# cuteboyqq/DPVO

Hardware: AMD Instinct MI355X
Metric: update-iterations/sec (altcorr+fastba) on 96-patch/2048-edge graph, 1→8 GPU (higher is better)
Workload: dtype f32; 1 GPU; cfg2: 96 patches/frame x 2048 edges, p=3, 4-level pyramid [1, 2, 4, 8], fp32 features, BA 2 iters; patches_per_frame=96, edges=2048, frames=12, radius=3, channels=128, feature_ring=36, parallelism=replicas x1

## Files before the change

dpvo_amd/csrc/ba_window.hip:

```cpp
#include <unistd.h>

#include <algorithm>
#include <chrono>
#include <cstdio>
#include <random>
#include <cstdlib>
#include <map>
#include <mutex>

#include "ba_paths.hpp"
#include "ba_solve.hpp"
#include "pyr_insert.hpp"

namespace dpvo {
namespace {
using namespace bad;

constexpr int kWT = 256;
constexpr int kPT = 512;
constexpr int kWMaxN = 16;
constexpr int kWMaxE = 10240;
constexpr int kWMaxG = 256;
constexpr int kWLds = 160 * 1024;
constexpr int kHistMax = 12288;
constexpr int kWSlots = 64;
constexpr unsigned kFix = 0xFF;
constexpr unsigned kHbm = 0xFE;
constexpr int kChunk = 256;
constexpr int kPart = 42;
constexpr int kPartPad = 48;
constexpr int kGranPad = 48;
constexpr long long kSpin = 2000000;
constexpr int kEpochWord = kWMaxG;
constexpr int kFlagWords = kWMaxG + 8;
constexpr int kRefine = 1;
constexpr int kBufDword3 = 0x00020000;
constexpr int kSc1 = 16;

constexpr int kStChol = 1, kStClamp = 2, kStTimeout = 16, kStCap = 32;

typedef unsigned v4u __attribute__((ext_vector_type(4)));

constexpr int kWMaxNB = kWMaxN * (kWMaxN + 1) / 2;
constexpr int kPlanShardMax = 16;
constexpr int kMetaWork = 64;
constexpr size_t kMetaBytes = sizeof(int) * (kMetaWork + (size_t)kPlanShardMax * kWMaxNB);

struct Plan {
  int* epos;
  int* poff;
  unsigned* pmask;
  int* pkk;
  int* meta;
  int* status;
  int* sink;
  const int* t0d;
};

struct WArgs {
  float* poses;
  float* patches;
  const float* intrinsics;
  const float* target;
  const float* weight;
  const float* lmbda;
  const int64_t* ii;
  const int64_t* jj;
  const int64_t* kk;
  int E, P, num_poses, num_patches, t0, N, iters, NB, Sd, So, G;
  Plan plan;
  double* part;
  v4u* gran;
  long long* flags;
  float* ejg;
  int* status;
  int* sink;
  int64_t* marks;
  double* dxo;
  const int* t0d;
  unsigned long long salt;
};

__device__ __forceinline__ size_t al16(size_t v) { return (v + 15) & ~(size_t)15; }
typedef double f64x2 __attribute__((ext_vector_type(2)));

__device__ __forceinline__ int opaque_tid() {
  int t = threadIdx.x;
  asm volatile("" : "+v"(t));
  return t;
}

__device__ __forceinline__ void mark(const WArgs& A, int slot) {
  if (A.marks && blockIdx.x == 0 && threadIdx.x == 0) A.marks[slot] = (int64_t)wall_clock64();
}


__host__ __device__ constexpr int plan_cap(int E) { return (E + 15) & ~15; }
__host__ __device__ constexpr size_t plan_u_bytes(int cap) {
  size_t p2 = 1;
  while (p2 < (size_t)cap) p2 <<= 1;
  const size_t keys = p2 <= 8192 ? 8 * p2 : 4 * p2;
  return keys > 8 * (size_t)cap ? keys : 8 * (size_t)cap;
}
__host__ __device__ constexpr size_t plan_lds_bytes(int cap) {
  return 256 + 6 * (size_t)cap + (((size_t)cap + 15) & ~(size_t)15) + plan_u_bytes(cap);
}
static_assert(plan_lds_bytes(kWMaxE) <= (size_t)kWLds, "plan LDS");

__device__ __forceinline__ int bucket_rank(const unsigned short* s, int a, int b, int e) {
  int rank = 0;
  for (int t = a; t < b; t += 8) {
    int v[8];
#pragma unroll
    for (int k = 0; k < 8; k++) v[k] = s[min(t + k, b - 1)];
#pragma unroll
    for (int k = 0; k < 8; k++) rank += (t + k < b && v[k] < e) ? 1 : 0;
  }
  return rank;
}

constexpr int kPlanPer = kWMaxE / kPT;
template <int kPer = kPlanPer>
__device__ __forceinline__ void plan_edges_pass(const int64_t* __restrict__ ii,
                                                const int64_t* __restrict__ jj,
                                                const int64_t* __restrict__ kk, int E,
                                                int num_patches, int num_poses, int t0, int N,
                                                int* ctl, unsigned short* code, int (&kv)[kPer]) {
  const int tid = threadIdx.x, lane = tid & 63, T = kPT;
  const int kmaxc = num_patches - 1;
  if (tid == 0) {
    ctl[0] = 0x7fffffff;
    ctl[1] = -1;
    ctl[2] = 0x7fffffff;
    ctl[3] = 0;
  }
  __syncthreads();
  constexpr int kPlanRound = kPer % 5 == 0 ? 5 : kPer;
  static_assert(kPer % kPlanRound == 0, "load rounds");
  int kmin = 0x7fffffff, kmax = -1, fmin = 0x7fffffff, bad = 0;
#pragma unroll
  for (int r = 0; r < kPer; r++) kv[r] = 0;
  if (E > 0) {
#pragma unroll
    for (int r0 = 0; r0 < kPer; r0 += kPlanRound) {
      if (r0 * T >= E) break;
      int64_t vk[kPlanRound], vi[kPlanRound], vj[kPlanRound];
#pragma unroll
      for (int r = 0; r < kPlanRound; r++) {
// ... 53 lines not shown
__device__ __forceinline__ void plan_store_work(const Plan& plan, const int* wl, int s, int N) {
  const int nb = N * (N + 1) / 2;
  for (int t = threadIdx.x; t < nb; t += blockDim.x)
    plan.meta[kMetaWork + t * kPlanShardMax + s] = wl[t];
}

__device__ __forceinline__ void plan_block(const int64_t* __restrict__ ii,
                                           const int64_t* __restrict__ jj,
                                           const int64_t* __restrict__ kk, int E, int num_patches,
                                           int num_poses, int t0, int N, const Plan& plan,
                                           char* lds, int cap = kWMaxE) {
  if (plan.t0d) t0 = *plan.t0d;
  const int tid = threadIdx.x, T = kPT;
  const int kmaxc = num_patches - 1;
  int* ctl = (int*)lds;
  int* scr = ctl + 16;
  unsigned short* code = (unsigned short*)(lds + 256);
  unsigned short* key = code + cap;
  unsigned short* spos = key + cap;
  unsigned char* head = (unsigned char*)(spos + cap);
  char* U = (char*)head + al16(cap);
  int kv[kPlanPer];
  plan_edges_pass(ii, jj, kk, E, num_patches, num_poses, t0, N, ctl, code, kv);
  int kmin = ctl[0];
  const int R = ctl[1] - kmin + 1;
  if (R <= kHistMax && (size_t)(R + E) * 4 <= plan_u_bytes(cap) && E < (1 << 14)) {
    int* hist = (int*)U;
    unsigned* pm = reinterpret_cast<unsigned*>(hist + R);
    for (int v = tid; v < R; v += T) hist[v] = 0;
    for (int u = tid; u < E; u += T) pm[u] = 0u;
    __syncthreads();
#pragma unroll
    for (int r = 0; r < kPlanPer; r++) {
      const int e = tid + r * T;
      if (e < E) atomicAdd(&hist[kv[r] - kmin], 1);
    }
    __syncthreads();
    const int nuniq = fscan(hist, R, scr, 14) & 0x3fff;
#pragma unroll
    for (int r = 0; r < kPlanPer; r++) {
      const int e = tid + r * T;
      if (e >= E) continue;
      const int old = atomicAdd(&hist[kv[r] - kmin], 1 << 14);
      spos[old >> 14] = (unsigned short)e;
      const unsigned c = code[e], ci = c & 0xff, cj = c >> 8;
      const unsigned m = (ci != kFix ? 1u << ci : 0u) | (cj != kFix ? 1u << cj : 0u);
      if (m) atomicOr(&pm[old & 0x3fff], m);
    }
    __syncthreads();
#pragma unroll
    for (int r = 0; r < kPlanPer; r++) {
      const int e = tid + r * T;
      if (e >= E) continue;
      const int v = kv[r] - kmin, hv = hist[v];
      const int b = hv >> 14, a = (v == 0) ? 0 : (hist[v - 1] >> 14);
      const int rank = bucket_rank(spos, a, b, e);
      plan.epos[a + rank] = e;
      if (rank == 0) {
        const int u = hv & 0x3fff;
        plan.poff[u] = a;
        plan.pkk[u] = kv[r];
        plan.pmask[u] = pm[u];
      }
    }
    if (tid == 0) {
      plan.poff[nuniq] = E;
      plan.meta[0] = nuniq;
      plan.meta[1] = ctl[2];
      plan.meta[2] = ctl[3];
      plan.meta[3] = 0;
      if (ctl[3] && plan.sink) atomicOr(plan.sink, ctl[3]);
      *plan.status = 0;
    }
    return;
  }
  unsigned short* pos_edge = spos;
  if (R <= kHistMax && (size_t)R * 4 <= plan_u_bytes(cap)) {
    int* hist = (int*)U;
    for (int v = tid; v < R; v += T) hist[v] = 0;
    for (int p = tid; p < E; p += T) head[p] = 0;
    __syncthreads();
#pragma unroll
    for (int r = 0; r < kPlanPer; r++) {
      const int e = tid + r * T;
      if (e < E) atomicAdd(&hist[kv[r] - kmin], 1);
    }
    __syncthreads();
    fscan(hist, R, scr);
    for (int v = tid; v < R; v += T) {
      const int a = hist[v], b = (v + 1 < R) ? hist[v + 1] : E;
      if (b > a) head[a] = 1;
    }
    __syncthreads();
#pragma unroll
    for (int r = 0; r < kPlanPer; r++) {
      const int e = tid + r * T;
      if (e < E) spos[atomicAdd(&hist[kv[r] - kmin], 1)] = (unsigned short)e;
    }
    __syncthreads();
    int dst[kPlanPer];
#pragma unroll
    for (int r = 0; r < kPlanPer; r++) {
      const int e = tid + r * T;
      dst[r] = -1;
      if (e >= E) continue;
      const int v = kv[r] - kmin;
      const int b = hist[v], a = (v == 0) ? 0 : hist[v - 1];
      dst[r] = a + bucket_rank(spos, a, b, e);
    }
    __syncthreads();
// ... 20 lines not shown
          k32[e] = ((unsigned)min(kv[r] - kmin, (1 << 18) - 1) << 14) | (unsigned)e;
      }
    }
    for (int i = E + tid; i < P2; i += T) {
      if (wide)
        k64[i] = ~0ull;
      else
        k32[i] = ~0u;
    }
    __syncthreads();
    for (int size = 2; size <= P2; size <<= 1)
      for (int stride = size >> 1; stride > 0; stride >>= 1) {
        for (int i = tid; i < P2 / 2; i += T) {
          const int lo = 2 * i - (i & (stride - 1));
          const int hi = lo + stride;
          const bool up = ((lo & size) == 0);
          if (wide) {
            const unsigned long long a = k64[lo], b = k64[hi];
            if ((a > b) == up) {
              k64[lo] = b;
              k64[hi] = a;
            }
          } else {
            const unsigned a = k32[lo], b = k32[hi];
            if ((a > b) == up) {
              k32[lo] = b;
              k32[hi] = a;
            }
          }
        }
        __syncthreads();
      }
    for (int p = tid; p < E; p += T) {
      if (wide) {
        spos[p] = (unsigned short)(k64[p] & 0xffffffffull);
        head[p] = (p == 0 || (k64[p] >> 32) != (k64[p - 1] >> 32)) ? 1 : 0;
      } else {
        spos[p] = (unsigned short)(k32[p] & 0x3fffu);
        head[p] = (p == 0 || (k32[p] >> 14) != (k32[p - 1] >> 14)) ? 1 : 0;
      }
    }
  }
  __syncthreads();
  int* hd = (int*)U;
  for (int p = tid; p < E; p += T) hd[p] = head[p];
  __syncthreads();
  const int nuniq = fscan(hd, E, scr);
  for (int p = tid; p < E; p += T) {
    const int u1 = (p + 1 < E) ? hd[p + 1] : nuniq;
    const bool is_head = u1 != hd[p];
    const int u = u1 - 1;
    const int e = pos_edge[p];
    plan.epos[p] = e;
    if (is_head) {
      plan.poff[u] = p;
      plan.pkk[u] = (int)min(max(kk[e], (int64_t)0), (int64_t)kmaxc);
    }
  }
  if (tid == 0) plan.poff[nuniq] = E;
  unsigned* mask = (unsigned*)(U + sizeof(int) * cap);
  for (int u = tid; u < nuniq; u += T) mask[u] = 0u;
  __syncthreads();
  for (int p = tid; p < E; p += T) {
    const int u = ((p + 1 < E) ? hd[p + 1] : nuniq) - 1;
    const unsigned c = code[pos_edge[p]];
    const unsigned ci = c & 0xff, cj = c >> 8;
    const unsigned m = (ci != kFix ? 1u << ci : 0u) | (cj != kFix ? 1u << cj : 0u);
    if (m) atomicOr(&mask[u], m);
  }
  __syncthreads();
  for (int u = tid; u < nuniq; u += T) plan.pmask[u] = mask[u];
  if (tid == 0) {
    plan.meta[0] = nuniq;
    plan.meta[1] = ctl[2];
    plan.meta[2] = ctl[3];
    plan.meta[3] = 0;
    if (ctl[3] && plan.sink) atomicOr(plan.sink, ctl[3]);
    *plan.status = 0;
  }
}

__host__ __device__ constexpr int plan_shards(int E) {
  return E <= 512 ? 1 : ((E + 511) / 512 < kPlanShardMax ? (E + 511) / 512 : kPlanShardMax);
}
template <int kPer>
__device__ __forceinline__ void plan_sharded_k(const int64_t* __restrict__ ii,
                                             const int64_t* __restrict__ jj,
                                               const int64_t* __restrict__ kk, int E, int num_patches,
                                               int num_poses, int t0, int N, const Plan& plan,
                                               char* lds, int cap, size_t lds_bytes, int s, int S) {
  if (S <= 1) {
    if (s == 0) plan_block(ii, jj, kk, E, num_patches, num_poses, t0, N, plan, lds, cap);
    return;
  }
  if (plan.t0d) t0 = *plan.t0d;
  auto stamp = [&](int q) {
    if (s == 0 && threadIdx.x == 0) {
      reinterpret_cast<int64_t*>(plan.meta + 16)[q] = (int64_t)wall_clock64();
      if (q == 0 || q == 6) reinterpret_cast<int64_t*>(plan.meta + 16)[7 + (q == 6)] = (int64_t)clock64();
    }
  };
  stamp(0);
  const int tid = threadIdx.x, lane = tid & 63, wid = tid >> 6, T = kPT;
  int* ctl = (int*)lds;
  int* scr = ctl + 16;
  unsigned short* spos = (unsigned short*)(lds + 256);
// ... 80 lines not shown
    }
    return;
  }
  const int lo = (int)((long long)R * s / S), hi = (int)((long long)R * (s + 1) / S), nl = hi - lo;
  const int per = (R + T - 1) / T, v0 = tid * per, v1 = min(v0 + per, R);
  int sum = 0;
  for (int k0 = v0; k0 < v1; k0 += 4) {
    int c[4];
#pragma unroll
    for (int j = 0; j < 4; j++) c[j] = hf[(kmin + min(k0 + j, v1 - 1)) & zm];
#pragma unroll
    for (int j = 0; j < 4; j++) sum += k0 + j < v1 ? (c[j] << 14) | (c[j] > 0 ? 1 : 0) : 0;
  }
  const int incl = wave_incl_sum(sum);
  if (lane == 63) scr[wid] = incl;
  lds_barrier();
  int total = 0, run = incl - sum;
#pragma unroll
  for (int w = 0; w < kPT / 64; w++) {
    const int x = scr[w];
    total += x;
    run += w < wid ? x : 0;
  }
  for (int k0 = v0; k0 < v1; k0 += 4) {
    int c[4];
#pragma unroll
    for (int j = 0; j < 4; j++) c[j] = hf[(kmin + min(k0 + j, v1 - 1)) & zm];
#pragma unroll
    for (int j = 0; j < 4; j++) {
      const int v = k0 + j;
      if (v >= v1) continue;
      if (v >= lo && v < hi) hf[(kmin + v) & zm] = run;
      if (v == lo) ctl[4] = run >> 14;
      if (v == hi) ctl[5] = run >> 14;
      run += (c[j] << 14) | (c[j] > 0 ? 1 : 0);
    }
  }
  lds_barrier();
  stamp(3);
  const int nuniq = total & 0x3fff;
  const int below = ctl[4], top = hi < R ? ctl[5] : total >> 14;
#pragma unroll
  for (int r = 0; r < kPer; r++) {
    const int e = tid + r * T;
    const int v = kv[r] - kmin - lo;
    if (e >= E || v < 0 || v >= nl) continue;
    const int p = atomicAdd(&hf[kv[r] & zm], 1 << 14) >> 14;
    spos[p] = (unsigned short)e;
    sv[p] = (unsigned short)v;
    if (mk[r]) atomicOr(&pm[v], mk[r]);
  }
  lds_barrier();
  stamp(4);
  plan_block_work(nl, [&](int v, int& c, unsigned& m) {
    c = (hf[(kmin + lo + v) & zm] >> 14) - (v == 0 ? below : (hf[(kmin + lo + v - 1) & zm] >> 14));
    m = pm[v];
  }, wl);
  stamp(5);
  for (int p = below + tid; p < top; p += T) {
    const int e = spos[p], v = sv[p];
    const int hv = hf[(kmin + lo + v) & zm];
    const int b = hv >> 14, a = v == 0 ? below : (hf[(kmin + lo + v - 1) & zm] >> 14);
    const int rank = bucket_rank(spos, a, b, e);
    plan.epos[a + rank] = e;
    if (rank == 0) {
      const int u = hv & 0x3fff;
      plan.poff[u] = a;
      plan.pkk[u] = kmin + lo + v;
      plan.pmask[u] = pm[v];
    }
  }
  lds_barrier();
  plan_store_work(plan, wl, s, N);
  if (tid == 0 && s == S - 1) plan.poff[nuniq] = E;
  if (tid == 0 && s == 0) {
    plan.meta[0] = nuniq;
    plan.meta[1] = ctl[2];
    plan.meta[2] = ctl[3];
    plan.meta[3] = S;
    if (ctl[3] && plan.sink) atomicOr(plan.sink, ctl[3]);
    *plan.status = 0;
  }
  stamp(6);
}

__device__ __forceinline__ void plan_sharded_long(const int64_t* __restrict__ ii,
                                               const int64_t* __restrict__ jj,
                                               const int64_t* __restrict__ kk, int E, int num_patches,
                                               int num_poses, int t0, int N, const Plan& plan,
                                               char* lds, int cap, size_t lds_bytes, int s, int S) {
  plan_sharded_k<kPlanPer>(ii, jj, kk, E, num_patches, num_poses, t0, N, plan, lds, cap, lds_bytes,
                           s, S);
}
__device__ __forceinline__ void plan_sharded(const int64_t* __restrict__ ii,
                                             const int64_t* __restrict__ jj,
                                             const int64_t* __restrict__ kk, int E, int num_patches,
                                             int num_poses, int t0, int N, const Plan& plan,
                                             char* lds, int cap, size_t lds_bytes, int s, int S) {
  if (__builtin_expect(E <= 4 * kPT, 1))
    plan_sharded_k<4>(ii, jj, kk, E, num_patches, num_poses, t0, N, plan, lds, cap, lds_bytes, s, S);
  else
    plan_sharded_long(ii, jj, kk, E, num_patches, num_poses, t0, N, plan, lds, cap, lds_bytes, s, S);
}

__global__ void __launch_bounds__(kPT) ba_plan_kernel(const int64_t* __restrict__ ii,
                                                      const int64_t* __restrict__ jj,
                                                      const int64_t* __restrict__ kk, int E,
                                                      int num_patches, int num_poses, int t0, int N,
                                                      Plan plan) {
  extern __shared__ __attribute__((aligned(16))) char lds[];
  plan_sharded(ii, jj, kk, E, num_patches, num_poses, t0, N, plan, lds, kWMaxE, kWLds, blockIdx.x,
               gridDim.x);
}

struct RArgs {
  const float* poses;
  const float* patches;
// ... 115 lines not shown
      const float4* e4 = reinterpret_cast<const float4*>(ej + 12 * (size_t)q);
      e0 = e4[0];
      e1 = e4[1];
      e2 = e4[2];
    } else {
      const __amdgpu_buffer_rsrc_t rs = __builtin_amdgcn_make_buffer_rsrc(
          const_cast<float*>(ejg), 0, (int)(sizeof(float) * 24 * (size_t)E), kBufDword3);
      const int o = (int)(sizeof(float) * 12 * ((size_t)par * E + eid[q]));
      e0 = __builtin_bit_cast(float4, __builtin_amdgcn_raw_buffer_load_b128(rs, o, 0, kSc1));
      e1 = __builtin_bit_cast(float4, __builtin_amdgcn_raw_buffer_load_b128(rs, o + 16, 0, kSc1));
      e2 = __builtin_bit_cast(float4, __builtin_amdgcn_raw_buffer_load_b128(rs, o + 32, 0, kSc1));
    }
  }
};

enum { cNrel = 0, cNrp = 1, cFmin = 2, cFail = 3, cTimeout = 4, cCap = 5, cFailAny = 6, cLMulti = 7,
       cScan = 16 };

__device__ __forceinline__ double edges_etdx(const WL& L, const WArgs& A, int q0, int q1, int par,
                                             int N) {
  constexpr int kEb = 4;
  double ex = 0.0;
  for (int qb = q0; qb < q1; qb += kEb) {
    float4 e[kEb][3];
    unsigned cc[kEb];
#pragma unroll
    for (int u = 0; u < kEb; u++) {
      const int q = min(qb + u, q1 - 1);
      cc[u] = L.ec[q];
      L.ld_ej(A.ejg, A.E, q, par, e[u][0], e[u][1], e[u][2]);
    }
#pragma unroll
    for (int u = 0; u < kEb; u++) {
      const bool live = qb + u < q1;
      const unsigned si = cc[u] & 0xff, sj = cc[u] >> 8;
      const unsigned nm = (unsigned)max(N - 1, 0);
      const double* dj = L.dX + 6 * min(sj, nm);
      const double* di = L.dX + 6 * min(si, nm);
      const float4 e0 = e[u][0], e1 = e[u][1], e2 = e[u][2];
      const double tj = (double)e0.x * dj[0] + (double)e0.y * dj[1] + (double)e0.z * dj[2] +
                        (double)e0.w * dj[3] + (double)e1.x * dj[4] + (double)e1.y * dj[5];
      const double ti = (double)e1.z * di[0] + (double)e1.w * di[1] + (double)e2.x * di[2] +
                        (double)e2.y * di[3] + (double)e2.z * di[4] + (double)e2.w * di[5];
      ex += (live && sj < (unsigned)N) ? tj : 0.0;
      ex += (live && si < (unsigned)N) ? ti : 0.0;
    }
  }
  return ex;
}
__device__ __forceinline__ double patch_etdx(const WL& L, const WArgs& A, int ri, int par, int N) {
  return edges_etdx(L, A, L.roff[ri], L.roff[ri + 1], par, N);
}

__device__ __forceinline__ unsigned wslot(int gp, int t0, int N, int fmin) {
  if (gp >= t0 && gp < t0 + N) return (unsigned)(gp - t0);
  const int k = gp - fmin;
  return (k >= 0 && k < kWSlots - N) ? (unsigned)(N + k) : kHbm;
}

__device__ __forceinline__ void pose_of(const WArgs& A, const WL& L, unsigned slot, int gp,
                                        float* P) {
  if (slot != kHbm) {
    const float4 a0 = *reinterpret_cast<const float4*>(L.pose + 8 * slot);
    const float4 a1 = *reinterpret_cast<const float4*>(L.pose + 8 * slot + 4);
    P[0] = a0.x; P[1] = a0.y; P[2] = a0.z; P[3] = a0.w; P[4] = a1.x; P[5] = a1.y; P[6] = a1.z;
  } else {
    const float* g = A.poses + 7 * (size_t)gp;
#pragma unroll
    for (int k = 0; k < 7; k++) P[k] = g[k];
  }
}

template <int MODE>
__device__ void assemble(const WArgs& A, const WL& L, int nrel, int a, int b, double lam,
                         float fx, float fy, float cx, float cy, int par, double* acc,
                         int& nact) {
  nact = 0;
  constexpr int NA = (MODE == 1) ? 27 : (MODE == 2 ? 36 : 1);
  const int tid = opaque_tid(), N = A.N;
  const unsigned ua = (unsigned)a, ub = (unsigned)b;
  double* pe = reinterpret_cast<double*>(L.region);
#pragma unroll
  for (int k = 0; k < NA; k++) acc[k] = 0.0;
  for (int pa = 0; pa < nrel;) {
    int pb = pa + 1;
    {
      int lo = pa + 1, hi = nrel;
      const int base = L.roff[pa];
      if (L.roff[nrel] - base <= kChunk) {
        lo = nrel;
      } else {
        while (lo < hi) {
          const int mid = (lo + hi + 1) >> 1;
          if (L.roff[mid] - base <= kChunk) lo = mid; else hi = mid - 1;
        }
      }
      pb = lo;
    }
    const int q0 = L.roff[pa], q1 = L.roff[pb];
    nact = max(nact, min(max(q1 - q0, pb - pa), kWT));
    for (int q = q0 + tid; q < q1; q += kWT) {
      const unsigned c = L.ec[q];
      const unsigned si = c & 0xff, sj = c >> 8;
      const int e = L.eid[q];
      float Pi[7], Pj[7];
      pose_of(A, L, si, si == kHbm ? (int)A.ii[e] : 0, Pi);
      pose_of(A, L, sj, sj == kHbm ? (int)A.jj[e] : 0, Pj);
      const int ri = L.rp[q];
      float4 tw;
      if (L.tw) {
        tw = L.tw[q];
      } else {
// ... 201 lines not shown
    double p0 = r[0] + r[1], p1 = r[2] + r[3], p2 = r[4] + r[5], p3 = r[6] + r[7];
    p0 += r[8] + r[9];
    p1 += r[10] + r[11];
    p2 += r[12] + r[13];
    p3 += r[14] + r[15];
    seg[t] = (p0 + p1) + (p2 + p3);
  }
  __syncthreads();
  if (tid < NA) {
    const double* s = seg + 8 * tid;
    const double v = ((s[0] + s[1]) + (s[2] + s[3])) + ((s[4] + s[5]) + (s[6] + s[7]));
    const __amdgpu_buffer_rsrc_t rs =
        __builtin_amdgcn_make_buffer_rsrc(gout, 0, 16 * kGranPad, kBufDword3);
    __builtin_amdgcn_raw_buffer_store_b128(granule(v, tag), rs, 16 * tid, 0, kSc1);
  }
}

__global__ void __launch_bounds__(kWT) ba_window_kernel(WArgs A) {
  extern __shared__ __attribute__((aligned(16))) char lds[];
  const int tid = threadIdx.x, g = blockIdx.x;
  const int N = A.N, P = A.P, PP = P * P, NB = A.NB;
  const float fx = A.intrinsics[0], fy = A.intrinsics[1], cx = A.intrinsics[2],
              cy = A.intrinsics[3];
  const int t0w = A.t0d ? *A.t0d : A.t0;
  const long long epoch =
      __hip_atomic_load(&A.flags[kEpochWord], __ATOMIC_RELAXED, __HIP_MEMORY_SCOPE_AGENT) + 1;
  mark(A, 0);

  WL L;
  L.ctl = (int*)lds;
  int* ctl = L.ctl;
  int* scr = ctl + cScan;
  L.pose = (float*)(lds + 256);
  L.dX = (double*)(lds + 256 + sizeof(float) * 8 * kWSlots);
  L.tri = (unsigned short*)(lds + 256 + sizeof(float) * 8 * kWSlots + sizeof(double) * 6 * kWMaxN);
  size_t off = al16(256 + sizeof(float) * 8 * kWSlots + sizeof(double) * 6 * kWMaxN +
                    sizeof(unsigned short) * (kWMaxN * (kWMaxN + 1) / 2));
  for (int t = tid; t < NB; t += kWT) {
    int ta, tb;
    tri_of(t, ta, tb);
    L.tri[t] = (unsigned short)((ta << 8) | tb);
  }
  constexpr int kB = 8;
  unsigned m0[kB];
  int pa0[kB], pb0[kB], kx0[kB];
#pragma unroll
  for (int r = 0; r < kB; r++) {
    const int u = min(tid + r * kWT, A.E - 1);
    m0[r] = A.plan.pmask[u];
    pa0[r] = A.plan.poff[u];
    pb0[r] = A.plan.poff[u + 1];
    kx0[r] = A.plan.pkk[u];
  }
  const int nuniq = A.plan.meta[0], fmin = A.plan.meta[1];
  int* bstart = reinterpret_cast<int*>(lds + off);
  off = al16(off + sizeof(int) * (kWMaxNB + 1));
  int* sdst = reinterpret_cast<int*>(lds + off);
  off = al16(off + sizeof(int) * kWMaxG);
  int* mlist = reinterpret_cast<int*>(lds + off);
  off = al16(off + sizeof(int) * kWMaxNB);
  for (int sl = tid; sl < A.G; sl += kWT) sdst[sl] = -1;
  const int gd = N * A.Sd, nlow = NB - N;
  const int gx = A.G - gd - nlow;
  int blk = 0, sub = 0, S = 1;
  if (NB > 0 && g < gd) {
    blk = g / A.Sd;
    sub = g - blk * A.Sd;
    S = A.Sd;
  }
  if (gx > 0 && nlow > 0) {
    const int lane = tid & 63;
    const int nsh = A.plan.meta[3];
    int w2[2];
#pragma unroll
    for (int h = 0; h < 2; h++) {
      const int o = min(2 * lane + h, nlow - 1);
      int ja = 1;
      while ((ja + 1) * ja / 2 <= o) ja++;
      const int4* src = reinterpret_cast<const int4*>(
          A.plan.meta + kMetaWork + (o + ja) * kPlanShardMax);
      int wq[kPlanShardMax];
#pragma unroll
      for (int q4 = 0; q4 < kPlanShardMax / 4; q4++) {
        const int4 v = src[q4];
        wq[4 * q4] = v.x;
        wq[4 * q4 + 1] = v.y;
        wq[4 * q4 + 2] = v.z;
        wq[4 * q4 + 3] = v.w;
      }
      int w = 0;
#pragma unroll
      for (int q = 0; q < kPlanShardMax; q++) w += q < nsh ? wq[q] : 0;
      w2[h] = (2 * lane + h < nlow) ? w : 0;
    }
    const int incl = wave_incl_sum(w2[0] + w2[1]);
    const int woff = __builtin_amdgcn_readlane(incl, 63);
    const bool prop = nsh > 0 && woff > 0;
    auto share0 = [&](int o, int cum) {
      return gd + (prop ? o + (int)((long long)gx * cum / woff) : o * A.So);
    };
    const int ex = incl - w2[0] - w2[1];
    const int st0 = share0(2 * lane, ex), st1 = share0(2 * lane + 1, ex + w2[0]);
    if (tid < 64) {
      if (2 * lane < nlow) bstart[N + 2 * lane] = st0;
      if (2 * lane + 1 < nlow) bstart[N + 2 * lane + 1] = st1;
    }
    if (g >= gd) {
      const unsigned long long b0 = __ballot(2 * lane < nlow && st0 <= g);
      const unsigned long long b1 = __ballot(2 * lane + 1 < nlow && st1 <= g);
      const int o = __popcll(b0) + __popcll(b1) - 1;
      const int s_o = __builtin_amdgcn_readlane((o & 1) ? st1 : st0, o >> 1);
      const int s_n = (o + 1 >= nlow) ? A.G
                                      : __builtin_amdgcn_readlane(((o + 1) & 1) ? st1 : st0,
                                                                  (o + 1) >> 1);
      blk = N + o;
      sub = g - s_o;
      S = s_n - s_o;
    }
  } else {
    if (tid > N && tid < NB) bstart[tid] = gd + (tid - N) * A.So;
    if (NB > 0 && g >= gd) {
      const int o = (g - gd) / A.So;
      blk = N + o;
      sub = g - gd - o * A.So;
      S = A.So;
    }
  }
  if (tid <= N) bstart[tid] = tid * A.Sd;
  if (tid == 0) bstart[NB] = A.G;
  int a = 0, b = 0;
  if (NB == 0) {
  } else if (blk < N) {
    a = b = blk;
  } else {
    const int o = blk - N;
    a = 1;
    while ((a + 1) * a / 2 <= o) a++;
    b = o - a * (a - 1) / 2;
  }
  const bool diag = (a == b);
  auto diag_shares = [&](int p) { return bstart[p + 1] - bstart[p]; };
  const unsigned need = (NB > 0) ? ((1u << a) | (1u << b)) : 0u;
  if (tid == 0) {
    ctl[cFail] = 0;
    ctl[cFailAny] = 0;
    ctl[cTimeout] = 0;
    ctl[cCap] = 0;
    ctl[cLMulti] = 0;
  }
  int* cnt = (int*)(lds + off);
  auto relevant = [&](unsigned m, int u) {
    return (NB == 0) ? true : (((m & need) == need && (u % S) == sub) || (g == 0 && m == 0));
  };
#pragma unroll
  for (int r = 0; r < kB; r++) {
    const int u = tid + r * kWT;
    if (u < nuniq) cnt[u] = relevant(m0[r], u) ? ((1 << 16) | (pb0[r] - pa0[r])) : 0;
  }
  for (int u0 = tid + kB * kWT; u0 < nuniq; u0 += kB * kWT) {
    unsigned m[kB];
    int p0[kB], p1[kB];
#pragma unroll
    for (int r = 0; r < kB; r++) {
      const int u = min(u0 + r * kWT, nuniq - 1);
      m[r] = A.plan.pmask[u];
      p0[r] = A.plan.poff[u];
      p1[r] = A.plan.poff[u + 1];
    }
#pragma unroll
    for (int r = 0; r < kB; r++) {
      const int u = u0 + r * kWT;
      if (u < nuniq) cnt[u] = relevant(m[r], u) ? ((1 << 16) | (p1[r] - p0[r])) : 0;
    }
  }
  mark(A, 40);
  __syncthreads();
  for (int o = tid; o < NB - N; o += kWT) {
    const int s0 = bstart[N + o], s1 = bstart[N + o + 1];
    int aa = 1;
    while ((aa + 1) * aa / 2 <= o) aa++;
    if (s1 - s0 == 1)
      sdst[s0] = 36 * (o + aa);
    else if (s1 - s0 > 1)
      mlist[atomicAdd(&ctl[cLMulti], 1)] = o | ((o + aa) << 16);
  }
  const int tot = fscan(cnt, nuniq, scr);
  mark(A, 41);
  int nrel = tot >> 16, nrp = tot & 0xffff;
  const size_t chunk_b = sizeof(double) * 2 * 14 * kChunk;
  const size_t red_b = sizeof(double) * (36 * 128 + 36 * 8);
  const size_t NN = N > 0 ? N : 1;
  const size_t solve_b =
      sizeof(double) * (36 * (NN * (NN + 1) / 2) + 6 * NN) + wsolve_bytes((int)NN) + 64;
  const size_t gather_b = sizeof(double) * (36 * (NN * (NN + 1) / 2) + 6 * NN + (size_t)kPartPad * A.G);
  size_t region_b = chunk_b > red_b ? chunk_b : red_b;
  region_b = region_b > solve_b ? region_b : solve_b;
  region_b = region_b > gather_b ? region_b : gather_b;
  const size_t rec0 = al16(off + sizeof(int) * (nuniq + 1));
  auto rec_bytes = [&](int nr, int ne) {
    return al16(sizeof(int) * (nr + 1)) + al16(sizeof(float2) * (nr + 1)) +
           2 * al16(sizeof(float) * (nr + 1)) + al16(sizeof(double2) * (nr + 1)) +
           al16(sizeof(int) * (nr + 1)) + 2 * al16(sizeof(unsigned short) * (ne + 1)) +
           al16(sizeof(int) * (ne + 1));
  };
  bool fits = rec0 + rec_bytes(nrel, nrp) + region_b <= (size_t)kWLds;
  if (!fits) {
    if (tid == 0) ctl[cCap] = 1;
    nrel = nrp = 0;
  }
  size_t o2 = rec0;
  auto take = [&](size_t bytes) {
    char* p = lds + o2;
    o2 = al16(o2 + bytes);
    return p;
  };
  L.roff = (int*)take(sizeof(int) * (nrel + 1));
  L.nxy = (float2*)take(sizeof(float2) * (nrel + 1));
  L.dep = (float*)take(sizeof(float) * (nrel + 1));
  L.dbase = (float*)take(sizeof(float) * (nrel + 1));
  L.qu = (double2*)take(sizeof(double2) * (nrel + 1));
  L.pkx = (int*)take(sizeof(int) * (nrel + 1));
  L.ec = (unsigned short*)take(sizeof(unsigned short) * (nrp + 1));
  L.rp = (unsigned short*)take(sizeof(unsigned short) * (nrp + 1));
  L.eid = (int*)take(sizeof(int) * (nrp + 1));
  L.region = take(region_b);
  const size_t tw_b = sizeof(float4) * (nrp + 1), ej_b = sizeof(float) * 12 * (nrp + 1);
  L.tw = nullptr;
  L.ej = nullptr;
  if (o2 + tw_b + ej_b <= (size_t)kWLds) {
    L.tw = (float4*)take(tw_b);
    L.ej = (float*)take(ej_b);
  } else if (o2 + tw_b <= (size_t)kWLds) {
    L.tw = (float4*)take(tw_b);
  }
  int* rpo = reinterpret_cast<int*>(L.qu);
  auto record = [&](int u, int kx, int po, unsigned m, int c0, int c1) {
    const int ri = c0 >> 16, q0 = c0 & 0xffff, ne = (c1 - c0) & 0xffff;
    L.roff[ri] = q0;
    rpo[ri] = po;
    for (int t = 0; t < ne; t++) L.rp[q0 + t] = (unsigned short)ri;
    if (ne > kChunk) ctl[cCap] = 1;
    bool own;
    if (NB == 0) own = true;
    else if (m == 0) own = (g == 0);
    else {
      unsigned mm = m;
      for (int t = (u >> 2) % __popc(m); t > 0; t--) mm &= mm - 1;
      const int po = __builtin_ctz(mm);
      own = diag && po == a && (u % diag_shares(po)) == sub;
    }
    L.pkx[ri] = own ? kx : -1;
    return ri;
  };
  auto cnt_at = [&](int u) { return (u < nuniq) ? cnt[u] : tot; };
  static_assert(kWMaxE <= 65536 && kWMaxN <= 16, "patch index and pose mask packed in 16 bits each");
  int* dl = rpo + (nrel + 1);
  bool lv0[kB];
  {
    int c0[kB], c1[kB];
#pragma unroll
    for (int r = 0; r < kB; r++) {
      const int u = min(tid + r * kWT, nuniq - 1);
      c0[r] = cnt[u];
      c1[r] = cnt_at(u + 1);
    }
#pragma unroll
    for (int r = 0; r < kB; r++) {
      const int u = tid + r * kWT;
      lv0[r] = nrel > 0 && u < nuniq && c0[r] != c1[r];
      if (lv0[r]) {
        int* d = dl + 3 * (c0[r] >> 16);
        d[0] = (int)((unsigned)u | (m0[r] << 16));
        d[1] = kx0[r];
        d[2] = pa0[r];
      }
    }
  }
  for (int u0 = tid + kB * kWT; u0 < nuniq && nrel > 0; u0 += kB * kWT) {
    int kx[kB], po[kB];
    unsigned msk[kB];
#pragma unroll
    for (int r = 0; r < kB; r++) {
      const int uc = min(u0 + r * kWT, nuniq - 1);
      kx[r] = A.plan.pkk[uc];
      po[r] = A.plan.poff[uc];
      msk[r] = A.plan.pmask[uc];
    }
    int c0[kB], c1[kB];
#pragma unroll
    for (int r = 0; r < kB; r++) {
      const int uc = min(u0 + r * kWT, nuniq - 1);
      c0[r] = cnt[uc];
      c1[r] = cnt_at(uc + 1);
    }
#pragma unroll
    for (int r = 0; r < kB; r++) {
      const int u = u0 + r * kWT;
      if (u < nuniq && c0[r] != c1[r]) {
        int* d = dl + 3 * (c0[r] >> 16);
        d[0] = (int)((unsigned)u | (msk[r] << 16));
        d[1] = kx[r];
        d[2] = po[r];
      }
    }
  }
  __syncthreads();
  const int c11 = P + 1;
  for (int t = tid; t < nrel; t += kWT) {
    const int* d = dl + 3 * t;
    const unsigned um = (unsigned)d[0];
    const int u = (int)(um & 0xffffu), kx = d[1];
    const float* pk = A.patches + (size_t)kx * 3 * PP;
    const float v0 = pk[c11], v1 = pk[PP + c11], v2 = pk[2 * PP + c11], v3 = pk[2 * PP];
    record(u, kx, d[2], um >> 16, cnt[u], cnt_at(u + 1));
    L.nxy[t] = make_float2((v0 - cx) / fx, (v1 - cy) / fy);
    L.dep[t] = v2;
    L.dbase[t] = v3;
  }
  if (tid == 0) L.roff[nrel] = nrp;
  __syncthreads();
  mark(A, 42);
  int ev0[kB];
#pragma unroll
  for (int r = 0; r < kB; r++) {
    const int q = min(tid + r * kWT, max(nrp - 1, 0));
    const int ri = nrp > 0 ? L.rp[q] : 0;
    const int p = nrp > 0 ? rpo[ri] + (q - L.roff[ri]) : 0;
    ev0[r] = A.plan.epos[min(max(p, 0), A.E - 1)];
  }
  constexpr int kPr = kWSlots * 8 / kWT;
  float pv[kPr];
#pragma unroll
  for (int r = 0; r < kPr; r++) {
    const int k = tid + r * kWT, sl = k >> 3, c = k & 7;
    const int gp = (sl < N) ? t0w + sl : fmin + (sl - N);
    pv[r] = A.poses[7 * (size_t)min(max(gp, 0), A.num_poses - 1) + min(c, 6)];
  }
#pragma unroll
  for (int r = 0; r < kPr; r++) {
    const int k = tid + r * kWT, sl = k >> 3, c = k & 7;
    const int gp = (sl < N) ? t0w + sl : fmin + (sl - N);
    const bool ok = c < 7 && gp >= 0 && gp < A.num_poses && (sl < N || fmin != 0x7fffffff);
    L.pose[k] = ok ? pv[r] : ((c == 6) ? 1.0f : 0.0f);
  }
  mark(A, 43);
  for (int q0 = tid; q0 < nrp; q0 += kB * kWT) {
    int ev[kB];
    if (q0 == tid) {
#pragma unroll
      for (int r = 0; r < kB; r++) ev[r] = ev0[r];
    } else {
#pragma unroll
      for (int r = 0; r < kB; r++) {
        const int q = min(q0 + r * kWT, nrp - 1);
        const int ri = L.rp[q];
        ev[r] = A.plan.epos[rpo[ri] + (q - L.roff[ri])];
      }
    }
    int64_t gi[kB], gj[kB];
    float2 tg[kB], wt[kB];
#pragma unroll
    for (int r = 0; r < kB; r++) {
      const int e = ev[r];
      gi[r] = A.ii[e];
      gj[r] = A.jj[e];
      tg[r] = reinterpret_cast<const float2*>(A.target)[e];
      wt[r] = reinterpret_cast<const float2*>(A.weight)[e];
    }
#pragma unroll
    for (int r = 0; r < kB; r++) {
      const int q = q0 + r * kWT;
      if (q >= nrp) continue;
      const unsigned si = wslot((int)gi[r], t0w, N, fmin), sj = wslot((int)gj[r], t0w, N, fmin);
      L.ec[q] = (unsigned short)(si | (sj << 8));
      L.eid[q] = ev[r];
      if (L.tw) L.tw[q] = make_float4(tg[r].x, tg[r].y, wt[r].x, wt[r].y);
    }
  }
  __syncthreads();
  mark(A, 1);
  if (A.marks && tid == 0 && g < 256) A.marks[kMarkSetup + g] = (int64_t)wall_clock64();
  const int nrel_e = nrel;

  const double lam = (double)A.lmbda[0];
  for (int it = 0; it < A.iters; it++) {
    const int tid = opaque_tid();
    const int mb = 2 + 8 * it;
    if (it > 0) {
      for (int i = tid; i < N; i += kWT) {
        float xi[6], tt[3], qq[4], t1[3], q1[4];
#pragma unroll
        for (int k = 0; k < 6; k++) xi[k] = (float)L.dX[6 * i + k];
        float* pl = L.pose + 8 * i;
        tt[0] = pl[0]; tt[1] = pl[1]; tt[2] = pl[2];
        qq[0] = pl[3]; qq[1] = pl[4]; qq[2] = pl[5]; qq[3] = pl[6];
        retrSE3(xi, tt, qq, t1, q1);
        pl[0] = t1[0]; pl[1] = t1[1]; pl[2] = t1[2];
        pl[3] = q1[0]; pl[4] = q1[1]; pl[5] = q1[2]; pl[6] = q1[3];
      }
      for (int ri = tid; ri < nrel_e; ri += kWT) {
        const double ex = patch_etdx(L, A, ri, (it - 1) & 1, N);
        const double2 qu = L.qu[ri];
        const float dz = (float)(qu.x * (qu.y - ex));
        const float base = (it == 1) ? L.dbase[ri] : L.dep[ri];
        float d = base + dz;
        d = (d > 20.0f) ? 1.0f : d;
        L.dep[ri] = (float)fmax((double)d, 1e-4);
      }
      __syncthreads();
    }
    double acc[36];
    int nact = kWT;
    double* red = reinterpret_cast<double*>(L.region);
    const unsigned long long gkey = (unsigned long long)(epoch * 64 + it + 1) ^ A.salt;
    const unsigned gtag = (unsigned)gkey;
    v4u* const gbuf = A.gran + (size_t)(it & 1) * A.G * kGranPad;
    v4u* const gslot = gbuf + (size_t)g * kGranPad;
    if (NB == 0) {
      assemble<0>(A, L, nrel_e, a, b, lam, fx, fy, cx, cy, it & 1, acc, nact);
    } else if (diag) {
      assemble<1>(A, L, nrel_e, a, b, lam, fx, fy, cx, cy, it & 1, acc, nact);
      mark(A, mb + 4);
      if (A.marks && tid == 0 && it == 0 && g < 256) A.marks[kMarkPre + g] = (int64_t)wall_clock64();
      reduce_acc<27>(acc, red, gslot, gkey, nact);
    } else {
      assemble<2>(A, L, nrel_e, a, b, lam, fx, fy, cx, cy, it & 1, acc, nact);
      if (A.marks && tid == 0 && it == 0 && g < 256) A.marks[kMarkPre + g] = (int64_t)wall_clock64();
      reduce_acc<36>(acc, red, gslot, gkey, nact);
    }
    mark(A, mb + 0);
// ... 229 lines not shown
    else if (w.So > 1) w.So--;
    else w.Sd--;
  }
  w.G = G();
  return w;
}

static int window_coresident() {
  static std::mutex mu;
  static std::map<int, int> cache;
  int dev = 0;
  if (hipGetDevice(&dev) != hipSuccess) return 0;
  std::lock_guard<std::mutex> lk(mu);
  auto it = cache.find(dev);
  if (it != cache.end()) return it->second;
  int cus = 0, per = 0;
  (void)hipFuncSetAttribute((const void*)ba_window_kernel,
                            hipFuncAttributeMaxDynamicSharedMemorySize, kWLds);
  if (hipDeviceGetAttribute(&cus, hipDeviceAttributeMultiprocessorCount, dev) != hipSuccess ||
      hipOccupancyMaxActiveBlocksPerMultiprocessor(&per, (const void*)ba_window_kernel, kWT,
                                                   kWLds) != hipSuccess) {
    (void)hipGetLastError();
    cus = per = 0;
  }
  cache[dev] = cus * per;
  return cache[dev];
}

static unsigned long long granule_salt() {
  static const unsigned long long salt = [] {
    unsigned long long v = 0;
    try {
      std::random_device rd;
      v = ((unsigned long long)rd() << 32) ^ rd();
    } catch (...) {
    }
    v ^= (unsigned long long)std::chrono::steady_clock::now().time_since_epoch().count() *
         0x9E3779B97F4A7C15ull;
    v ^= (unsigned long long)getpid() << 17;
    return v;
  }();
  return salt;
}

bool ba_window_supported(int E, int N, int P) {
  if (E <= 0 || E > kWMaxE || N < 0 || N > kWMaxN || P < 2 || P * P > 64) return false;
  const int G = window_grid(E, N).G;
  return G <= kWMaxG && G <= window_coresident();
}

static size_t gran_count(int G) { return (size_t)2 * kGranPad * G; }

struct WScratch {
  size_t epos, poff, pmask, pkk, meta;
  size_t part, gran, ejg;
  size_t bytes;
};
static WScratch window_scratch(int E, int G) {
  WScratch s;
  size_t off = 0;
  auto take = [&off](size_t bytes) {
    const size_t at = off;
    off += al256w(bytes);
    return at;
  };
  s.epos = take(sizeof(int) * (size_t)E);
  s.poff = take(sizeof(int) * (size_t)(E + 1));
  s.pmask = take(sizeof(unsigned) * (size_t)E);
  s.pkk = take(sizeof(int) * (size_t)E);
  s.meta = take(kMetaBytes);
  s.part = take(sizeof(double) * 2 * kPartPad * (size_t)G);
  s.gran = take((size_t)16 * gran_count(G));
  s.ejg = take(sizeof(float) * 24 * (size_t)E);
  s.bytes = off;
  return s;
}

size_t ba_window_scratch_bytes(int E, int N) {
  return window_scratch(E, window_grid(E, N).G).bytes;
}

namespace {
std::mutex g_wflag_mu;
std::map<int, long long*> g_wflags;
long long* wflag_slot(hipStream_t st) {
  int dev = 0;
  (void)hipGetDevice(&dev);
  std::lock_guard<std::mutex> lk(g_wflag_mu);
  auto it = g_wflags.find(dev);
  if (it != g_wflags.end()) return it->second;
  long long* p = nullptr;
  if (hipMalloc(&p, sizeof(long long) * kFlagWords) != hipSuccess) return nullptr;
  if (hipMemsetAsync(p, 0, sizeof(long long) * kFlagWords, st) != hipSuccess) return nullptr;
  g_wflags[dev] = p;
  return p;
}
}

namespace {
std::mutex g_sink_mu;
std::map<int, int*> g_sink;
int* sink_for_device() {
  int dev = 0;
  (void)hipGetDevice(&dev);
  std::lock_guard<std::mutex> lk(g_sink_mu);
  auto it = g_sink.find(dev);
  return it == g_sink.end() ? nullptr : it->second;
}
}

void ba_set_status_sink(int* sink) {
  int dev = 0;
  (void)hipGetDevice(&dev);
  std::lock_guard<std::mutex> lk(g_sink_mu);
  g_sink[dev] = sink;
}

void ba_window_plan_offsets(int E, int64_t* out) {
  const WScratch s = window_scratch(E, 0);
  const size_t o[5] = {s.epos, s.poff, s.pmask, s.pkk, s.meta};
  for (int k = 0; k < 5; k++) out[k] = (int64_t)o[k];
}

static Plan plan_view(const BaProblem& p, const BaWindowWs& ws) {
  const WScratch s = window_scratch(p.E, 0);
  Plan v;
  v.epos = (int*)(ws.scratch + s.epos);
  v.poff = (int*)(ws.scratch + s.poff);
  v.pmask = (unsigned*)(ws.scratch + s.pmask);
  v.pkk = (int*)(ws.scratch + s.pkk);
  v.meta = (int*)(ws.scratch + s.meta);
  v.status = ws.status;
  v.sink = sink_for_device();
  v.t0d = p.t0d;
  return v;
}

static RArgs reproject_args(const BaProblem& p, int N2, float* coords, int* order,
                            int64_t* marks) {
  RArgs r;
  r.marks = marks;
  r.poses = p.poses;
  r.patches = p.patches;
  r.intrinsics = p.intrinsics;
  r.ii = p.ii;
  r.jj = p.jj;
  r.kk = p.kk;
  r.E = p.E;
  r.P = p.P;
  r.num_poses = p.num_poses;
  r.num_patches = p.num_patches;
  r.N2 = N2;
  r.t0 = p.t0;
  r.N = p.N;
  r.coords = coords;
  r.order = order;
  r.nps = plan_shards(p.E);
  r.spread = 0;
  return r;
}

static void set_attrs() {
  static bool attr = false;
  if (!attr) {
    (void)hipFuncSetAttribute((const void*)ba_window_kernel,
                              hipFuncAttributeMaxDynamicSharedMemorySize, kWLds);
    (void)hipFuncSetAttribute((const void*)ba_plan_kernel,
                              hipFuncAttributeMaxDynamicSharedMemorySize, kWLds);
    (void)hipFuncSetAttribute((const void*)reproject_plan_kernel,
                              hipFuncAttributeMaxDynamicSharedMemorySize, kWLds);
    (void)hipFuncSetAttribute((const void*)reproject_plan_insert_kernel<float>,
                              hipFuncAttributeMaxDynamicSharedMemorySize, kWLds);
    (void)hipFuncSetAttribute((const void*)reproject_plan_insert_kernel<__half>,
                              hipFuncAttributeMaxDynamicSharedMemorySize, kWLds);
    attr = true;
  }
}

int ba_window_plan(const BaProblem& p, const BaWindowWs& ws, void* stream) {
  set_attrs();
  hipLaunchKernelGGL(ba_plan_kernel, dim3(plan_shards(p.E)), dim3(kPT), kWLds, as_stream(stream),
                     p.ii, p.jj, p.kk, p.E, p.num_patches, p.num_poses, p.t0, p.N,
                     plan_view(p, ws));
  return launch_status();
// ... 90 lines not shown
```

Before: 8933 update-iterations/s.

## Precompute edge pose slots in plan and replace LDS scan with wave-level prefix sums

```diff
diff --git a/dpvo_amd/csrc/ba_window.hip b/dpvo_amd/csrc/ba_window.hip
--- a/dpvo_amd/csrc/ba_window.hip
+++ b/dpvo_amd/csrc/ba_window.hip
@@ -51,6 +51,7 @@
   int* poff;
   unsigned* pmask;
   int* pkk;
+  unsigned short* pslot;
   int* meta;
   int* status;
   int* sink;
@@ -94,6 +95,18 @@
   if (A.marks && blockIdx.x == 0 && threadIdx.x == 0) A.marks[slot] = (int64_t)wall_clock64();
 }
 
+
+__device__ __forceinline__ unsigned wslot(int gp, int t0, int N, int fmin) {
+  if (gp >= t0 && gp < t0 + N) return (unsigned)(gp - t0);
+  const int k = gp - fmin;
+  return (k >= 0 && k < kWSlots - N) ? (unsigned)(N + k) : kHbm;
+}
+__device__ __forceinline__ unsigned short pslot_of(int gi, int gj, int t0, int N, int fmin) {
+  return (unsigned short)(wslot(gi, t0, N, fmin) | (wslot(gj, t0, N, fmin) << 8));
+}
+__device__ __forceinline__ int low_word(const int64_t* x, int e) {
+  return reinterpret_cast<const int*>(x)[2 * (size_t)e];
+}
 
 __host__ __device__ constexpr int plan_cap(int E) { return (E + 15) & ~15; }
 __host__ __device__ constexpr size_t plan_u_bytes(int cap) {
@@ -253,10 +266,12 @@
     for (int r = 0; r < kPlanPer; r++) {
       const int e = tid + r * T;
       if (e >= E) continue;
+      const int gi = low_word(ii, e), gj = low_word(jj, e);
       const int v = kv[r] - kmin, hv = hist[v];
       const int b = hv >> 14, a = (v == 0) ? 0 : (hist[v - 1] >> 14);
       const int rank = bucket_rank(spos, a, b, e);
       plan.epos[a + rank] = e;
+      plan.pslot[a + rank] = pslot_of(gi, gj, t0, N, ctl[2]);
       if (rank == 0) {
         const int u = hv & 0x3fff;
         plan.poff[u] = a;
@@ -383,6 +398,7 @@
     const int u = u1 - 1;
     const int e = pos_edge[p];
     plan.epos[p] = e;
+    plan.pslot[p] = pslot_of(low_word(ii, e), low_word(jj, e), t0, N, ctl[2]);
     if (is_head) {
       plan.poff[u] = p;
       plan.pkk[u] = (int)min(max(kk[e], (int64_t)0), (int64_t)kmaxc);
@@ -569,6 +585,8 @@
   }
   lds_barrier();
   stamp(4);
+  const int e_first = min((int)spos[min(below + tid, cap - 1)], E - 1);
+  int gi = low_word(ii, e_first), gj = low_word(jj, e_first);
   plan_block_work(nl, [&](int v, int& c, unsigned& m) {
     c = (hf[(kmin + lo + v) & zm] >> 14) - (v == 0 ? below : (hf[(kmin + lo + v - 1) & zm] >> 14));
     m = pm[v];
@@ -576,10 +594,15 @@
   stamp(5);
   for (int p = below + tid; p < top; p += T) {
     const int e = spos[p], v = sv[p];
+    if (p != below + tid) {
+      gi = low_word(ii, e);
+      gj = low_word(jj, e);
+    }
     const int hv = hf[(kmin + lo + v) & zm];
     const int b = hv >> 14, a = v == 0 ? below : (hf[(kmin + lo + v - 1) & zm] >> 14);
     const int rank = bucket_rank(spos, a, b, e);
     plan.epos[a + rank] = e;
+    plan.pslot[a + rank] = pslot_of(gi, gj, t0, N, ctl[2]);
     if (rank == 0) {
       const int u = hv & 0x3fff;
       plan.poff[u] = a;
@@ -801,12 +824,6 @@
   return edges_etdx(L, A, L.roff[ri], L.roff[ri + 1], par, N);
 }
 
-__device__ __forceinline__ unsigned wslot(int gp, int t0, int N, int fmin) {
-  if (gp >= t0 && gp < t0 + N) return (unsigned)(gp - t0);
-  const int k = gp - fmin;
-  return (k >= 0 && k < kWSlots - N) ? (unsigned)(N + k) : kHbm;
-}
-
 __device__ __forceinline__ void pose_of(const WArgs& A, const WL& L, unsigned slot, int gp,
                                         float* P) {
   if (slot != kHbm) {
@@ -1114,6 +1131,13 @@
     pb0[r] = A.plan.poff[u + 1];
     kx0[r] = A.plan.pkk[u];
   }
+  constexpr int kPr = kWSlots * 8 / kWT;
+  float pvf[kPr];
+#pragma unroll
+  for (int r = 0; r < kPr; r++) {
+    const int k = tid + r * kWT, sl = k >> 3, c = k & 7;
+    pvf[r] = A.poses[7 * (size_t)min(max(t0w + sl, 0), A.num_poses - 1) + min(c, 6)];
+  }
   const int nuniq = A.plan.meta[0], fmin = A.plan.meta[1];
   int* bstart = reinterpret_cast<int*>(lds + off);
   off = al16(off + sizeof(int) * (kWMaxNB + 1));
@@ -1210,29 +1234,45 @@
     ctl[cCap] = 0;
     ctl[cLMulti] = 0;
   }
-  int* cnt = (int*)(lds + off);
+  static_assert(kWT == 256 && kB * (kWT / 64) == 32 && cScan + 32 <= 64,
+                "the first batch's (slot, wave) totals fill ctl[cScan, cScan + 32)");
+  constexpr int kBatch = kB * kWT, kTot = kB * (kWT / 64);
+  constexpr int kXBatch = (kWMaxE + kBatch - 1) / kBatch - 1;
+  int* wtx = (int*)(lds + off);
+  int* xs = wtx + kXBatch * kTot;
+  static_assert(kXBatch * kTot <= kBatch, "wtx + xs lie inside the nuniq + 1 ints before the records");
+  const int lane_s = tid & 63, wid_s = tid >> 6;
   auto relevant = [&](unsigned m, int u) {
     return (NB == 0) ? true : (((m & need) == need && (u % S) == sub) || (g == 0 && m == 0));
   };
+  int x0[kB];
+  unsigned relb = 0;
 #pragma unroll
   for (int r = 0; r < kB; r++) {
     const int u = tid + r * kWT;
-    if (u < nuniq) cnt[u] = relevant(m0[r], u) ? ((1 << 16) | (pb0[r] - pa0[r])) : 0;
-  }
-  for (int u0 = tid + kB * kWT; u0 < nuniq; u0 += kB * kWT) {
+    const int cv = (u < nuniq && relevant(m0[r], u)) ? ((1 << 16) | (pb0[r] - pa0[r])) : 0;
+    const int incl = wave_incl_sum(cv);
+    x0[r] = incl - cv;
+    relb |= cv ? (1u << r) : 0u;
+    if (lane_s == 63) scr[r * (kWT / 64) + wid_s] = incl;
+  }
+  for (int ub = kBatch, bx = 0; ub < nuniq; ub += kBatch, bx++) {
     unsigned m[kB];
     int p0[kB], p1[kB];
 #pragma unroll
     for (int r = 0; r < kB; r++) {
-      const int u = min(u0 + r * kWT, nuniq - 1);
+      const int u = min(ub + tid + r * kWT, nuniq - 1);
       m[r] = A.plan.pmask[u];
       p0[r] = A.plan.poff[u];
       p1[r] = A.plan.poff[u + 1];
     }
 #pragma unroll
     for (int r = 0; r < kB; r++) {
-      const int u = u0 + r * kWT;
-      if (u < nuniq) cnt[u] = relevant(m[r], u) ? ((1 << 16) | (p1[r] - p0[r])) : 0;
+      const int u = ub + tid + r * kWT;
+      const int cv = (u < nuniq && relevant(m[r], u)) ? ((1 << 16) | (p1[r] - p0[r])) : 0;
+      const int incl = wave_incl_sum(cv);
+      if (u < nuniq) xs[u - kBatch] = incl - cv;
+      if (lane_s == 63) wtx[bx * kTot + r * (kWT / 64) + wid_s] = incl;
     }
   }
   mark(A, 40);
@@ -1246,7 +1286,21 @@
     else if (s1 - s0 > 1)
       mlist[atomicAdd(&ctl[cLMulti], 1)] = o | ((o + aa) << 16);
   }
-  const int tot = fscan(cnt, nuniq, scr);
+  int base0[kB], tot = 0;
+#pragma unroll
+  for (int r = 0; r < kB; r++) {
+    const int4 w4 = *reinterpret_cast<const int4*>(scr + r * (kWT / 64));
+    const int w[4] = {w4.x, w4.y, w4.z, w4.w};
+    base0[r] = tot;
+#pragma unroll
+    for (int k = 0; k < 4; k++) {
+      base0[r] += k < wid_s ? w[k] : 0;
+      tot += w[k];
+    }
+  }
+  const int tot1 = tot;
+  for (int ub = kBatch, bx = 0; ub < nuniq; ub += kBatch, bx++)
+    for (int k = 0; k < kTot; k++) tot += wtx[bx * kTot + k];
   mark(A, 41);
   int nrel = tot >> 16, nrp = tot & 0xffff;
   const size_t chunk_b = sizeof(double) * 2 * 14 * kChunk;
@@ -1296,8 +1350,7 @@
     L.tw = (float4*)take(tw_b);
   }
   int* rpo = reinterpret_cast<int*>(L.qu);
-  auto record = [&](int u, int kx, int po, unsigned m, int c0, int c1) {
-    const int ri = c0 >> 16, q0 = c0 & 0xffff, ne = (c1 - c0) & 0xffff;
+  auto record = [&](int ri, int u, int kx, int po, unsigned m, int q0, int ne) {
     L.roff[ri] = q0;
     rpo[ri] = po;
     for (int t = 0; t < ne; t++) L.rp[q0 + t] = (unsigned short)ri;
@@ -1314,118 +1367,129 @@
     L.pkx[ri] = own ? kx : -1;
     return ri;
   };
-  auto cnt_at = [&](int u) { return (u < nuniq) ? cnt[u] : tot; };
   static_assert(kWMaxE <= 65536 && kWMaxN <= 16, "patch index and pose mask packed in 16 bits each");
   int* dl = rpo + (nrel + 1);
-  bool lv0[kB];
+  int2* dq = reinterpret_cast<int2*>(L.nxy);
+  if (nrel > 0) {
+#pragma unroll
+    for (int r = 0; r < kB; r++) {
+      if (!((relb >> r) & 1u)) continue;
+      const int c0 = base0[r] + x0[r], ri = c0 >> 16;
+      int* d = dl + 3 * ri;
+      d[0] = (int)((unsigned)(tid + r * kWT) | (m0[r] << 16));
+      d[1] = kx0[r];
+      d[2] = pa0[r];
+      dq[ri] = make_int2(c0 & 0xffff, pb0[r] - pa0[r]);
+    }
+  }
   {
-    int c0[kB], c1[kB];
-#pragma unroll
-    for (int r = 0; r < kB; r++) {
-      const int u = min(tid + r * kWT, nuniq - 1);
-      c0[r] = cnt[u];
-      c1[r] = cnt_at(u + 1);
-    }
-#pragma unroll
-    for (int r = 0; r < kB; r++) {
-      const int u = tid + r * kWT;
-      lv0[r] = nrel > 0 && u < nuniq && c0[r] != c1[r];
-      if (lv0[r]) {
-        int* d = dl + 3 * (c0[r] >> 16);
-        d[0] = (int)((unsigned)u | (m0[r] << 16));
-        d[1] = kx0[r];
-        d[2] = pa0[r];
-      }
-    }
-  }
-  for (int u0 = tid + kB * kWT; u0 < nuniq && nrel > 0; u0 += kB * kWT) {
-    int kx[kB], po[kB];
-    unsigned msk[kB];
-#pragma unroll
-    for (int r = 0; r < kB; r++) {
-      const int uc = min(u0 + r * kWT, nuniq - 1);
-      kx[r] = A.plan.pkk[uc];
-      po[r] = A.plan.poff[uc];
-      msk[r] = A.plan.pmask[uc];
-    }
-    int c0[kB], c1[kB];
-#pragma unroll
-    for (int r = 0; r < kB; r++) {
-      const int uc = min(u0 + r * kWT, nuniq - 1);
-      c0[r] = cnt[uc];
-      c1[r] = cnt_at(uc + 1);
-    }
-#pragma unroll
-    for (int r = 0; r < kB; r++) {
-      const int u = u0 + r * kWT;
-      if (u < nuniq && c0[r] != c1[r]) {
-        int* d = dl + 3 * (c0[r] >> 16);
-        d[0] = (int)((unsigned)u | (msk[r] << 16));
-        d[1] = kx[r];
-        d[2] = po[r];
+    int run = tot1;
+    for (int ub = kBatch, bx = 0; ub < nuniq && nrel > 0; ub += kBatch, bx++) {
+      int kx[kB], po[kB], p1[kB];
+      unsigned msk[kB];
+#pragma unroll
+      for (int r = 0; r < kB; r++) {
+        const int uc = min(ub + tid + r * kWT, nuniq - 1);
+        kx[r] = A.plan.pkk[uc];
+        po[r] = A.plan.poff[uc];
+        p1[r] = A.plan.poff[uc + 1];
+        msk[r] = A.plan.pmask[uc];
+      }
+#pragma unroll
+      for (int r = 0; r < kB; r++) {
+        const int u = ub + tid + r * kWT;
+        int base = run;
+#pragma unroll
+        for (int k = 0; k < kWT / 64; k++) {
+          const int w = wtx[bx * kTot + r * (kWT / 64) + k];
+          base += k < wid_s ? w : 0;
+          run += w;
+        }
+        if (u < nuniq && relevant(msk[r], u)) {
+          const int c0 = base + xs[u - kBatch], ri = c0 >> 16;
+          int* d = dl + 3 * ri;
+          d[0] = (int)((unsigned)u | (msk[r] << 16));
+          d[1] = kx[r];
+          d[2] = po[r];
+          dq[ri] = make_int2(c0 & 0xffff, p1[r] - po[r]);
+        }
       }
     }
   }
   __syncthreads();
   const int c11 = P + 1;
-  for (int t = tid; t < nrel; t += kWT) {
+  float v0 = 0.0f, v1 = 0.0f, v2 = 0.0f, v3 = 0.0f;
+  if (tid < nrel) {
+    const int* d = dl + 3 * tid;
+    const unsigned um = (unsigned)d[0];
+    const int kx = d[1];
+    const int2 qn = dq[tid];
+    const float* pk = A.patches + (size_t)kx * 3 * PP;
+    v0 = pk[c11], v1 = pk[PP + c11], v2 = pk[2 * PP + c11], v3 = pk[2 * PP];
+    record(tid, (int)(um & 0xffffu), kx, d[2], um >> 16, qn.x, qn.y);
+  }
+  for (int t = tid + kWT; t < nrel; t += kWT) {
     const int* d = dl + 3 * t;
     const unsigned um = (unsigned)d[0];
-    const int u = (int)(um & 0xffffu), kx = d[1];
+    const int kx = d[1];
+    const int2 qn = dq[t];
     const float* pk = A.patches + (size_t)kx * 3 * PP;
-    const float v0 = pk[c11], v1 = pk[PP + c11], v2 = pk[2 * PP + c11], v3 = pk[2 * PP];
-    record(u, kx, d[2], um >> 16, cnt[u], cnt_at(u + 1));
-    L.nxy[t] = make_float2((v0 - cx) / fx, (v1 - cy) / fy);
-    L.dep[t] = v2;
-    L.dbase[t] = v3;
+    const float w0 = pk[c11], w1 = pk[PP + c11], w2 = pk[2 * PP + c11], w3 = pk[2 * PP];
+    record(t, (int)(um & 0xffffu), kx, d[2], um >> 16, qn.x, qn.y);
+    L.nxy[t] = make_float2((w0 - cx) / fx, (w1 - cy) / fy);
+    L.dep[t] = w2;
+    L.dbase[t] = w3;
   }
   if (tid == 0) L.roff[nrel] = nrp;
-  __syncthreads();
+  lds_barrier();
   mark(A, 42);
   int ev0[kB];
+  unsigned ps0[kB];
 #pragma unroll
   for (int r = 0; r < kB; r++) {
     const int q = min(tid + r * kWT, max(nrp - 1, 0));
     const int ri = nrp > 0 ? L.rp[q] : 0;
     const int p = nrp > 0 ? rpo[ri] + (q - L.roff[ri]) : 0;
-    ev0[r] = A.plan.epos[min(max(p, 0), A.E - 1)];
-  }
-  constexpr int kPr = kWSlots * 8 / kWT;
-  float pv[kPr];
+    const int pc = min(max(p, 0), A.E - 1);
+    ev0[r] = A.plan.epos[pc];
+    ps0[r] = A.plan.pslot[pc];
+  }
+  float pvx[kPr];
 #pragma unroll
   for (int r = 0; r < kPr; r++) {
     const int k = tid + r * kWT, sl = k >> 3, c = k & 7;
-    const int gp = (sl < N) ? t0w + sl : fmin + (sl - N);
-    pv[r] = A.poses[7 * (size_t)min(max(gp, 0), A.num_poses - 1) + min(c, 6)];
-  }
-#pragma unroll
-  for (int r = 0; r < kPr; r++) {
-    const int k = tid + r * kWT, sl = k >> 3, c = k & 7;
-    const int gp = (sl < N) ? t0w + sl : fmin + (sl - N);
-    const bool ok = c < 7 && gp >= 0 && gp < A.num_poses && (sl < N || fmin != 0x7fffffff);
-    L.pose[k] = ok ? pv[r] : ((c == 6) ? 1.0f : 0.0f);
+    const int gp = fmin != 0x7fffffff ? fmin + (sl - N) : 0;
+    pvx[r] = A.poses[7 * (size_t)min(max(gp, 0), A.num_poses - 1) + min(c, 6)];
+  }
+  if (tid < nrel) {
+    L.nxy[tid] = make_float2((v0 - cx) / fx, (v1 - cy) / fy);
+    L.dep[tid] = v2;
+    L.dbase[tid] = v3;
   }
   mark(A, 43);
   for (int q0 = tid; q0 < nrp; q0 += kB * kWT) {
     int ev[kB];
+    unsigned ps[kB];
     if (q0 == tid) {
 #pragma unroll
-      for (int r = 0; r < kB; r++) ev[r] = ev0[r];
+      for (int r = 0; r < kB; r++) {
+        ev[r] = ev0[r];
+        ps[r] = ps0[r];
+      }
     } else {
 #pragma unroll
       for (int r = 0; r < kB; r++) {
         const int q = min(q0 + r * kWT, nrp - 1);
         const int ri = L.rp[q];
-        ev[r] = A.plan.epos[rpo[ri] + (q - L.roff[ri])];
-      }
-    }
-    int64_t gi[kB], gj[kB];
+        const int p = rpo[ri] + (q - L.roff[ri]);
+        ev[r] = A.plan.epos[p];
+        ps[r] = A.plan.pslot[p];
+      }
+    }
     float2 tg[kB], wt[kB];
 #pragma unroll
     for (int r = 0; r < kB; r++) {
       const int e = ev[r];
-      gi[r] = A.ii[e];
-      gj[r] = A.jj[e];
       tg[r] = reinterpret_cast<const float2*>(A.target)[e];
       wt[r] = reinterpret_cast<const float2*>(A.weight)[e];
     }
@@ -1433,11 +1497,17 @@
     for (int r = 0; r < kB; r++) {
       const int q = q0 + r * kWT;
       if (q >= nrp) continue;
-      const unsigned si = wslot((int)gi[r], t0w, N, fmin), sj = wslot((int)gj[r], t0w, N, fmin);
-      L.ec[q] = (unsigned short)(si | (sj << 8));
+      L.ec[q] = (unsigned short)ps[r];
       L.eid[q] = ev[r];
       if (L.tw) L.tw[q] = make_float4(tg[r].x, tg[r].y, wt[r].x, wt[r].y);
     }
+  }
+#pragma unroll
+  for (int r = 0; r < kPr; r++) {
+    const int k = tid + r * kWT, sl = k >> 3, c = k & 7;
+    const int gp = (sl < N) ? t0w + sl : (fmin != 0x7fffffff ? fmin + (sl - N) : -1);
+    const bool ok = c < 7 && gp >= 0 && gp < A.num_poses;
+    L.pose[k] = ok ? (sl < N ? pvf[r] : pvx[r]) : ((c == 6) ? 1.0f : 0.0f);
   }
   __syncthreads();
   mark(A, 1);
@@ -1773,7 +1843,7 @@
 static size_t gran_count(int G) { return (size_t)2 * kGranPad * G; }
 
 struct WScratch {
-  size_t epos, poff, pmask, pkk, meta;
+  size_t epos, poff, pmask, pkk, meta, pslot;
   size_t part, gran, ejg;
   size_t bytes;
 };
@@ -1790,6 +1860,7 @@
   s.pmask = take(sizeof(unsigned) * (size_t)E);
   s.pkk = take(sizeof(int) * (size_t)E);
   s.meta = take(kMetaBytes);
+  s.pslot = take(sizeof(unsigned short) * (size_t)E);
   s.part = take(sizeof(double) * 2 * kPartPad * (size_t)G);
   s.gran = take((size_t)16 * gran_count(G));
   s.ejg = take(sizeof(float) * 24 * (size_t)E);
@@ -1851,6 +1922,7 @@
   v.pmask = (unsigned*)(ws.scratch + s.pmask);
   v.pkk = (int*)(ws.scratch + s.pkk);
   v.meta = (int*)(ws.scratch + s.meta);
+  v.pslot = (unsigned short*)(ws.scratch + s.pslot);
   v.status = ws.status;
   v.sink = sink_for_device();
   v.t0d = p.t0d;
```

Result: faster. 9091 update-iterations/s (median of 6 runs) (+1.8%).
